# ericbrec/BSpy

Hardware: AMD Instinct MI355X
Metric: M evals/sec on 10M-point bicubic (p=3x3) surface (higher is better)
Workload: dtype f64; 1 GPU; BASELINE configs[1]: bicubic surface order 4x4, nCoef 64x64, nDep 3, fp64, clamped uniform knots, Spline.evaluate on 10000000 uniform-random (u,v); points_total=10000000, points_per_gpu=10000000, op=evaluate

## Files before the change

bspy_amd/csrc/bsk_api.hip:

```cpp
#include "bsk_kernels.hpp"
#include "bsk_tile.hpp"
#include "bsk_stream.hpp"
#include "bsk_rowrot.hpp"
#include "bsk_uniform.hpp"
#include "bsk_rec32.hpp"
#include "bsk_host.hpp"

#include <condition_variable>
#include <mutex>
#include <thread>

struct HostPipe;
static void pipe_destroy(HostPipe *p);

static int ceil_log2(int x)
{
    int s = 0;
    while ((1 << s) < x) ++s;
    return s;
}

template <typename T>
static void build_axis_table(const T *knots, int order, int nk, std::vector<T> &tab)
{
// ... 198 lines not shown
    };
#define HIPCHK_C(expr)                                                                        \
    do {                                                                                      \
        hipError_t e_ = (expr);                                                               \
        if (e_ != hipSuccess) {                                                               \
            cleanup();                                                                        \
            return fail(BSK_ERR_HIP, std::string(#expr) + ": " + hipGetErrorString(e_));      \
        }                                                                                     \
    } while (0)
    HIPCHK_C(hipSetDevice(device));
    hipDeviceProp_t prop;
    HIPCHK_C(hipGetDeviceProperties(&prop, device));
    s->num_cu = prop.multiProcessorCount > 0 ? prop.multiProcessorCount : 256;
    s->lds_max = std::min<size_t>(160 * 1024, prop.maxSharedMemoryPerMultiProcessor > 0
                                                  ? (size_t)prop.maxSharedMemoryPerMultiProcessor
                                                  : (size_t)64 * 1024);
    HIPCHK_C(hipMalloc(&s->tab, std::max<size_t>(16, s->esize * (size_t)tab_len)));
    HIPCHK_C(hipMalloc(&s->coef, std::max<size_t>(16, s->esize * (size_t)coef_len)));
    {
        const size_t tbytes = s->esize * (size_t)tab_len + s->esize * (size_t)coef_len;
        int omax = 0;
        for (int iv = 0; iv < nInd; ++iv) omax = std::max(omax, order[iv]);
        bool fixed = nInd <= 3 && omax <= 6;
        if (fixed && nDep <= 4 && tbytes + 8192 > s->lds_max)
            HIPCHK_C(hipMalloc(&s->coef_aos, std::max<size_t>(16, s->esize * (size_t)coef_len)));
        else if (fixed && nDep <= 4 && nInd == 2 && !s->same_order && omax >= 2) {
            HIPCHK_C(hipMalloc(&s->coef_aos, std::max<size_t>(16, s->esize * (size_t)coef_len)));
            s->aos_small = true;
        }
    }
    HIPCHK_C(hipMalloc((void **)&s->lut, std::max<size_t>(16, sizeof(unsigned) * (size_t)(dtype == BSK_F32 ? s->t32.lut_len : s->t64.lut_len))));
    HIPCHK_C(hipMalloc((void **)&s->bad, sizeof(unsigned long long)));
    if (const char *v = getenv("BSK_VARIANT")) s->variant = atoi(v);
    HIPCHK_C(hipMemset(s->bad, 0xff, sizeof(unsigned long long)));
#undef HIPCHK_C
    st = dtype == BSK_F32 ? upload_tables<float>(s, knots, coefs) : upload_tables<double>(s, knots, coefs);
    if (st == BSK_OK) st = dtype == BSK_F32 ? upload_uniform<float>(s, knots, coefs) : upload_uniform<double>(s, knots, coefs);
    if (st == BSK_OK) st = dtype == BSK_F32 ? upload_uniform_nd<float>(s, knots, coefs) : upload_uniform_nd<double>(s, knots, coefs);
    if (st != BSK_OK) { s->uni_img.release(); cleanup(); return st; }
    *out = s;
    return BSK_OK;
}

extern "C" bsk_status bsk_spline_update(bsk_spline s, const void *const *knots, const void *coefs)
{
    if (!s || !knots || !coefs) return fail(BSK_ERR_INVALID, "NULL argument");
    HIPCHK(hipSetDevice(s->device));
    HIPCHK(hipDeviceSynchronize());
    const bsk_status st = s->dtype == BSK_F32 ? upload_tables<float>(s, knots, coefs) : upload_tables<double>(s, knots, coefs);
    if (st != BSK_OK) return st;
    const bsk_status su = s->dtype == BSK_F32 ? upload_uniform<float>(s, knots, coefs) : upload_uniform<double>(s, knots, coefs);
    if (su != BSK_OK) return su;
    return s->dtype == BSK_F32 ? upload_uniform_nd<float>(s, knots, coefs) : upload_uniform_nd<double>(s, knots, coefs);
}

extern "C" bsk_status bsk_spline_destroy(bsk_spline s)
{
    if (!s) return BSK_OK;
    (void)hipSetDevice(s->device);
    (void)hipDeviceSynchronize();
    if (s->tab) (void)hipFree(s->tab);
    if (s->coef) (void)hipFree(s->coef);
    if (s->bad) (void)hipFree(s->bad);
    if (s->lut) (void)hipFree(s->lut);
    if (s->coef_aos) (void)hipFree(s->coef_aos);
    s->in_ws.release();
// ... 383 lines not shown
    std::vector<unsigned char> img(total_b, 0);
    for (int iv = 0; iv < nInd; ++iv)
        memcpy(img.data() + un.kn_off[iv], static_cast<const T *>(knots[iv]) + O - 1, (size_t)(un.ns[iv] + 1) * sizeof(T));
    T *ic = reinterpret_cast<T *>(img.data() + un.coef_off);
    for (size_t i = 0; i < w.size(); ++i) ic[i] = T(w[i]);
    HIPCHK(hipSetDevice(s->device));
    HIPCHK(s->uni_img.reserve(total_b));
    HIPCHK(hipMemcpy(s->uni_img.p, img.data(), total_b, hipMemcpyHostToDevice));
    s->uniN = true;
    return BSK_OK;
}

template <typename T, bool NORMAL>
static bsk_status launch_jac_rowrot(bsk_spline s, const Params<T> &prm, long long n, T *out, int normalize, int negate,
                                    hipStream_t st)
{
    const Desc<T> &d = desc_of<T>(s);
    const TileDesc<T> &tdr = tile_of<T>(s);
    const size_t lds_rr = rowrot_lds_bytes<T>(s);
    const T *tab = static_cast<const T *>(s->tab);
    const T *coef = static_cast<const T *>(s->coef);
    const int per_cu = (int)std::max<size_t>(1, std::min<size_t>(2, s->lds_max / lds_rr));
    if (s->uni) {
        const UniDesc<T> &ud = uni_of<T>(s);
        const size_t lds_u = (size_t)ud.img_bytes + TILE * sizeof(unsigned);
        const int per_cu_u = (int)std::max<size_t>(1, std::min<size_t>(2, s->lds_max / lds_u));
#define BSK_JUNI(O_, ND_)                                                                                               \
    do {                                                                                                                 \
        s->last_kernel = "jac_uni";                                        \
        HIPCHK(allow_lds(jac_uni<T, O_, NORMAL, ND_>, lds_u));                                                          \
        hipLaunchKernelGGL((jac_uni<T, O_, NORMAL, ND_>), dim3(g), dim3(TILE), lds_u, st, ud, s->uni_img.p, cp,         \
                           (unsigned)m, n0, out + n0, n, s->bad, normalize, negate);                                    \
    } while (0)
        const int ndu = (NORMAL || s->nDep > 3) ? 0 : s->nDep;
        const long long cmaxu = rr_chunk_points();
        for (long long n0 = 0; n0 < n; n0 += cmaxu) {
            const long long m = std::min<long long>(n - n0, cmaxu);
            const int g = (int)std::max<long long>(1, std::min<long long>((m + TILE - 1) / TILE, (long long)s->num_cu * per_cu_u));
            Params<T> cp = prm;
            for (int iv = 0; iv < s->nInd; ++iv) cp.p[iv] = prm.p[iv] + n0;
            if (s->order[0] == 4) {
                if constexpr (NORMAL) BSK_JUNI(4, 3);
                else switch (ndu) { case 1: BSK_JUNI(4, 1); break; case 2: BSK_JUNI(4, 2); break; case 3: BSK_JUNI(4, 3); break; default: BSK_JUNI(4, 0); }
            } else {
                if constexpr (NORMAL) BSK_JUNI(2, 3);
                else switch (ndu) { case 1: BSK_JUNI(2, 1); break; case 2: BSK_JUNI(2, 2); break; case 3: BSK_JUNI(2, 3); break; default: BSK_JUNI(2, 0); }
            }
            HIPCHK(hipGetLastError());
        }
#undef BSK_JUNI
        return BSK_OK;
    }
#define BSK_JROT(O_, ND_)                                                                                               \
    do {                                                                                                                 \
        s->last_kernel = "jac_rowrot";                                        \
        HIPCHK(allow_lds(jac_rowrot<T, O_, NORMAL, ND_>, lds_rr));                                                      \
        hipLaunchKernelGGL((jac_rowrot<T, O_, NORMAL, ND_>), dim3(g), dim3(TILE), lds_rr, st, d, tdr, tab, s->lut, coef, \
                           cp, (unsigned)m, n0, out + n0, n, s->bad, normalize, negate);                                \
    } while (0)
    const int nd = (NORMAL || s->nDep > 3) ? 0 : s->nDep;
    const long long cmax = rr_chunk_points();
    for (long long n0 = 0; n0 < n; n0 += cmax) {
        const long long m = std::min<long long>(n - n0, cmax);
        const int g = (int)std::max<long long>(1, std::min<long long>((m + TILE - 1) / TILE, (long long)s->num_cu * per_cu));
        Params<T> cp = prm;
        for (int iv = 0; iv < s->nInd; ++iv) cp.p[iv] = prm.p[iv] + n0;
        if (s->order[0] == 4) {
            if constexpr (NORMAL) BSK_JROT(4, 0);
            else switch (nd) { case 1: BSK_JROT(4, 1); break; case 2: BSK_JROT(4, 2); break; case 3: BSK_JROT(4, 3); break; default: BSK_JROT(4, 0); }
        } else {
            if constexpr (NORMAL) BSK_JROT(2, 0);
            else switch (nd) { case 1: BSK_JROT(2, 1); break; case 2: BSK_JROT(2, 2); break; case 3: BSK_JROT(2, 3); break; default: BSK_JROT(2, 0); }
        }
        HIPCHK(hipGetLastError());
    }
#undef BSK_JROT
    return BSK_OK;
}

template <typename T, int NIND, int O>
static bsk_status launch_eval_lds(bsk_spline s, size_t lds, const Params<T> &prm, long long n, T *out, long long ostride,
                                  const Wrt &w, hipStream_t st)
{
    const Desc<T> &d = desc_of<T>(s);
    const TileDesc<T> &td = tile_of<T>(s);
    const T *tab = static_cast<const T *>(s->tab);
    const T *coef = static_cast<const T *>(s->coef);
    bool deriv = false;
    for (int iv = 0; iv < s->nInd; ++iv) deriv |= w.w[iv] != 0;
    const long long ntiles = (n + TILE - 1) / TILE;
    if constexpr (NIND == 2 && (O == 2 || O == 4)) {
        if (rowrot_applies<T>(s)) {
            if (s->uni) {
                const UniDesc<T> &ud = uni_of<T>(s);
                const size_t lds_u = (size_t)ud.img_bytes + TILE * sizeof(unsigned);
                const int per_cu_u = (int)std::max<size_t>(1, std::min<size_t>(2, s->lds_max / lds_u));
#define BSK_UNI(DERIV_, ND_)                                                                                             \
    do {                                                                                                                 \
        s->last_kernel = "eval_uni";                                        \
        HIPCHK(allow_lds(eval_uni<T, O, DERIV_, ND_>, lds_u));                                                          \
        hipLaunchKernelGGL((eval_uni<T, O, DERIV_, ND_>), dim3(g), dim3(TILE), lds_u, st, ud, s->uni_img.p, cp,         \
                           (unsigned)m, n0, out + n0, ostride, w, s->bad);                                              \
    } while (0)
#define BSK_UNI_ND(DERIV_)                                                                                               \
    switch (s->nDep) {                                                                                                   \
    case 1: BSK_UNI(DERIV_, 1); break;                                                                                   \
    case 2: BSK_UNI(DERIV_, 2); break;                                                                                   \
    case 3: BSK_UNI(DERIV_, 3); break;                                                                                   \
    default: BSK_UNI(DERIV_, 0); break;                                                                                  \
    }
                const long long cmaxu = rr_chunk_points();
                for (long long n0 = 0; n0 < n; n0 += cmaxu) {
                    const long long m = std::min<long long>(n - n0, cmaxu);
                    const int g = (int)std::max<long long>(1, std::min<long long>((m + TILE - 1) / TILE, (long long)s->num_cu * per_cu_u));
                    Params<T> cp = prm;
                    for (int iv = 0; iv < s->nInd; ++iv) cp.p[iv] = prm.p[iv] + n0;
                    if (deriv) { BSK_UNI_ND(true); } else { BSK_UNI_ND(false); }
                    HIPCHK(hipGetLastError());
                }
#undef BSK_UNI_ND
#undef BSK_UNI
                return BSK_OK;
            }
            if constexpr (sizeof(T) == 4 && O == 4) {
                const size_t lds_r = r32_lds_bytes(s->ncoef[0] - 3, s->ncoef[1] - 3, td.lut_len, s->ncoef[0], s->ncoef[1]);
                if (s->variant == 0 && s->nDep >= 1 && s->nDep <= 4 && lds_r + 256 <= s->lds_max) {
                    const int per_cu_r = (int)std::max<size_t>(1, std::min<size_t>(2, s->lds_max / lds_r));
#define BSK_R32(DERIV_, ND_)                                                                                             \
    do {                                                                                                                 \
        HIPCHK(allow_lds(eval_rec32<DERIV_, ND_>, lds_r));                                                              \
        hipLaunchKernelGGL((eval_rec32<DERIV_, ND_>), dim3(g), dim3(TILE), lds_r, st, d, td, tab, s->lut, coef, cp,     \
                           (unsigned)m, n0, out + n0, ostride, w, s->bad);                                              \
    } while (0)
#define BSK_R32_ND(DERIV_)                                                                                               \
    switch (s->nDep) {                                                                                                   \
    case 1: BSK_R32(DERIV_, 1); break;                                                                                   \
    case 2: BSK_R32(DERIV_, 2); break;                                                                                   \
    case 3: BSK_R32(DERIV_, 3); break;                                                                                   \
    default: BSK_R32(DERIV_, 4); break;                                                                                  \
    }
                    s->last_kernel = "eval_rec32";
                    const long long cmaxr = rr_chunk_points();
                    for (long long n0 = 0; n0 < n; n0 += cmaxr) {
                        const long long m = std::min<long long>(n - n0, cmaxr);
                        const int g = (int)std::max<long long>(1, std::min<long long>((m + TILE - 1) / TILE, (long long)s->num_cu * per_cu_r));
                        Params<T> cp = prm;
                        for (int iv = 0; iv < s->nInd; ++iv) cp.p[iv] = prm.p[iv] + n0;
                        if (deriv) { BSK_R32_ND(true); } else { BSK_R32_ND(false); }
                        HIPCHK(hipGetLastError());
                    }
#undef BSK_R32_ND
#undef BSK_R32
                    return BSK_OK;
// ... 1341 lines not shown
```

bspy_amd/csrc/bsk_host.hpp:

```cpp
#pragma once
#include <algorithm>
#include <cmath>
#include <cstdio>
#include <cstring>
#include <limits>
#include <string>
#include <tuple>
#include <vector>

#include "bsk_common.hpp"
#include "bsk_tile.hpp"

using namespace bsk;

inline thread_local std::string g_err;

inline bsk_status fail(bsk_status st, const std::string &msg)
{
    g_err = msg;
    return st;
}

#define HIPCHK(expr)                                                                          \
    do {                                                                                      \
// ... 10 lines not shown
        if (bytes <= cap) return hipSuccess;
        if (p) (void)hipFree(p);
        p = nullptr;
        cap = 0;
        hipError_t e = hipMalloc(&p, bytes);
        if (e == hipSuccess) cap = bytes;
        return e;
    }
    void release()
    {
        if (p) (void)hipFree(p);
        p = nullptr;
        cap = 0;
    }
};

struct bsk_spline_s {
    bsk_dtype dtype;
    int device;
    int nInd, nDep;
    int order[MAXI], ncoef[MAXI];
    bool same_order;
    bool aos_small = false;
    size_t esize;
    Desc<float> d32;
    Desc<double> d64;
    TileDesc<float> t32;
    TileDesc<double> t64;
    void *tab = nullptr;
    void *coef = nullptr;
    void *coef_aos = nullptr;
    unsigned *lut = nullptr;
    int variant = 0;
    unsigned long long *bad = nullptr;
    int num_cu = 256;
    size_t lds_max = 160 * 1024;
    DevBuf in_ws, out_ws, aux_ws;
    DevBuf bin_ws;
    unsigned *ticket = nullptr;
    bool bin_reuse = false;
    DevBuf curv_ws;
    std::vector<unsigned char> tab_host;
    void *pin = nullptr;
    size_t pin_cap = 0;
    struct HostPipe *pipe = nullptr;
    bool uni = false;
    UniDesc<float> u32;
    UniDesc<double> u64;
    DevBuf uni_img;
    bool uniN = false;
    UniDescN<float> un32;
    UniDescN<double> un64;
    const char *last_kernel = "";
    static constexpr int MAX_STAGES = 12;
    bool stage_timing = false;
    hipEvent_t stage_ev[MAX_STAGES] = {};
    const char *stage_name[MAX_STAGES] = {};
    int stage_count = 0;
};

inline void stage_mark(bsk_spline s, hipStream_t st, const char *name, bool first = false)
{
    if (!s->stage_timing) return;
    if (first) s->stage_count = 0;
    if (s->stage_count >= bsk_spline_s::MAX_STAGES) return;
    hipEvent_t &e = s->stage_ev[s->stage_count];
// ... 58 lines not shown
```

bspy_amd/csrc/bsk_uniform.hpp:

```cpp
#pragma once
#include "bsk_rowrot.hpp"

namespace bsk {

__device__ __forceinline__ void stage_linear(char *smem, const void *__restrict__ gimg, unsigned bytes)
{
    const uint4 *__restrict__ g = static_cast<const uint4 *>(gimg);
    uint4 *s = reinterpret_cast<uint4 *>(smem);
    const unsigned n16 = bytes >> 4;
    constexpr int U = 8;
    const unsigned bd = blockDim.x;
    for (unsigned i0 = threadIdx.x; i0 < n16; i0 += bd * U) {
        uint4 v[U];
#pragma unroll
        for (int k = 0; k < U; ++k) v[k] = g[min(i0 + k * bd, n16 - 1u)];
#pragma unroll
        for (int k = 0; k < U; ++k) { const unsigned i = i0 + k * bd; if (i < n16) s[i] = v[k]; }
    }
}

template <typename T, bool NANFIX>
__device__ __forceinline__ void uni_spans2(const unsigned (&kn_a)[2], const UniDesc<T> &ud, const T (&u)[2], int (&m)[2],
                                           T (&z)[2])
{
    int m0[2];
    T t1[2];
#pragma unroll
    for (int iv = 0; iv < 2; ++iv) {
        const T x = (u[iv] - ud.lo[iv]) * ud.inv_h[iv] - ud.eps;
        m0[iv] = min(max((int)x, 0), ud.ns[iv] - 1);
        t1[iv] = LdsRead<T>::template at<(int)sizeof(T)>(kn_a[iv] + (unsigned)m0[iv] * (unsigned)sizeof(T));
    }
    lds_wait_n<0, 2>(t1);
#pragma unroll
    for (int iv = 0; iv < 2; ++iv) {
        const bool inc = (u[iv] >= t1[iv]) & (m0[iv] < ud.ns[iv] - 1);
        m[iv] = m0[iv] + (inc ? 1 : 0);
        z[iv] = (u[iv] - t1[iv]) * ud.inv_h[iv] + (inc ? T(0) : T(1));
        if (NANFIX && u[iv] != u[iv]) m[iv] = ud.ns[iv] - 1;
    }
}

template <typename T, int O, bool DERIV>
__device__ __forceinline__ void uni_basis(T z, int wrt, T inv_h, T (&b)[O])
{
#pragma unroll
    for (int k = 0; k < O; ++k) b[k] = T(0);
    b[O - 1] = T(1);
#pragma unroll
    for (int D = 1; D < O; ++D) {
        if (!DERIV || D < O - wrt) {
            if (D == 1) {
                b[O - 2] = T(1) - z;
                b[O - 1] = z;
            } else {
                const T rD = T(1.0 / (double)D);
#pragma unroll
                for (int j = 0; j < D; ++j) {
                    const int bi = O - D + j;
                    const T alpha = (z + T(D - 1 - j)) * rD;
                    b[bi - 1] += (T(1) - alpha) * b[bi];
                    b[bi] *= alpha;
                }
            }
        } else {
#pragma unroll
            for (int j = 0; j < D; ++j) {
                const int bi = O - D + j;
                b[bi - 1] -= inv_h * b[bi];
                b[bi] *= inv_h;
            }
        }
    }
// ... 176 lines not shown
        __builtin_amdgcn_s_setprio(3);
#pragma unroll
        for (int dep = 0; dep < nDep; ++dep) {
            T c[O][O];
            if constexpr (ND > 0) {
                uni_issue_window<T, O, ND>(ra, dep, c);
            } else {
#pragma unroll
                for (int a = 0; a < O; ++a) lds_issue_row<T, O>(ra[a], c[a]);
            }
            block_wait<0>(c);
            T q[O];
#pragma unroll
            for (int a = 0; a < O; ++a) {
                T t = T(0);
#pragma unroll
                for (int k = 0; k < O; ++k) t += c[a][k] * b[1][k];
                q[a] = mul_rn<T>(t, b0r[a]);
            }
            T r;
            if constexpr (O == 2) r = add_rn<T>(q[0], q[1]);
            else r = add_rn<T>(add_rn<T>(q[0], q[2]), add_rn<T>(q[1], q[3]));
            rr_store(o, off, r);
            o += ostride;
            if constexpr (ND == 0) {
#pragma unroll
                for (int a = 0; a < O; ++a) ra[a] += dstride;
            }
        }
        __builtin_amdgcn_s_setprio(0);
    }
}

template <typename T, int O, bool NORMAL, int ND>
__global__ __launch_bounds__(TILE) void jac_uni(const UniDesc<T> ud, const void *__restrict__ gimg, const Params<T> prm,
                                                const unsigned N, const long long n0, T *__restrict__ out,
                                                const long long ostride, unsigned long long *bad, const int normalize,
                                                const int negate)
{
    static_assert(O == 2 || O == 4, "row rotation covers orders 2 and 4");
    static_assert(!NORMAL || ND == 3, "the fused normal is a surface in 3-D");
    constexpr int CS = ND > 0 ? ND : 1;
    extern __shared__ __attribute__((aligned(16))) char smem[];
    const unsigned kn_a[2] = {(unsigned)(size_t)smem + ud.kn_off[0], (unsigned)(size_t)smem + ud.kn_off[1]};
    const unsigned coef_a = (unsigned)(size_t)smem + ud.coef_off;
    const int rs = ud.rs;
    const unsigned rstride = (unsigned)rs * (unsigned)sizeof(T);
    const unsigned dstride = (unsigned)(ud.ncoef[0] * rs) * (unsigned)sizeof(T);
    const int lane = threadIdx.x & 63;
    const unsigned stride = gridDim.x * (unsigned)TILE;
    unsigned n = ((threadIdx.x >> 6) * gridDim.x + blockIdx.x) * 64u + (unsigned)lane;
    const T lo0 = ud.lo[0], lo1 = ud.lo[1], hi0 = ud.hi[0], hi1 = ud.hi[1];
    const T *p0 = prm.p[0], *p1 = prm.p[1];
    T un[2] = {lo0, lo1};
    if (n < N) { un[0] = rr_load(p0, n * (unsigned)sizeof(T)); un[1] = rr_load(p1, n * (unsigned)sizeof(T)); }
    stage_linear(smem, gimg, ud.img_bytes);
    __syncthreads();
    unsigned *s_rc = reinterpret_cast<unsigned *>(smem + ud.img_bytes) + (threadIdx.x & ~63);
    asm volatile("" : "+v"(un[0]), "+v"(un[1]));
    const int ndep = ND > 0 ? ND : ud.nDep;

    for (; n < N; n += stride) {
        const T u[2] = {un[0], un[1]};
        const bool outside = (u[0] < lo0) | (u[0] > hi0) | (u[1] < lo1) | (u[1] > hi1);
        {
            const unsigned nn = min(n + stride, N - 1u) * (unsigned)sizeof(T);
// ... 48 lines not shown
                dv = add_rn<T>(add_rn<T>(qv[0], qv[2]), add_rn<T>(qv[1], qv[3]));
            }
            if constexpr (NORMAL) {
                if (dep == 0) { su[0] = du; sv[0] = dv; }
                else if (dep == 1) { su[1] = du; sv[1] = dv; }
                else { su[2] = du; sv[2] = dv; }
            } else {
                rr_store(o, off, du);
                rr_store(o + ostride, off, dv);
                o += 2 * ostride;
            }
            if constexpr (ND == 0) {
#pragma unroll
                for (int a = 0; a < O; ++a) ra[a] += dstride;
            }
        }
        __builtin_amdgcn_s_setprio(0);
        if constexpr (NORMAL) {
            T nx = su[1] * sv[2] - sv[1] * su[2];
            T ny = -(su[0] * sv[2] - sv[0] * su[2]);
            T nz = su[0] * sv[1] - sv[0] * su[1];
            if (negate) { nx = -nx; ny = -ny; nz = -nz; }
            if (normalize) {
                const T inv = T(1) / sqrt(nx * nx + ny * ny + nz * nz);
                nx = nx * inv; ny = ny * inv; nz = nz * inv;
            }
            rr_store(out, off, nx);
            rr_store(out + ostride, off, ny);
            rr_store(out + 2 * ostride, off, nz);
        }
    }
}

template <typename T, int NIND, bool NANFIX>
__device__ __forceinline__ void uni_spans(unsigned img_a, const UniDescN<T> &un, const T (&u)[NIND], int (&m)[NIND], T (&z)[NIND])
{
    int m0[NIND];
    T t1[NIND];
#pragma unroll
    for (int iv = 0; iv < NIND; ++iv) {
        const T x = (u[iv] - un.lo[iv]) * un.inv_h[iv] - un.eps;
        m0[iv] = min(max((int)x, 0), un.ns[iv] - 1);
        t1[iv] = LdsRead<T>::template at<(int)sizeof(T)>(img_a + un.kn_off[iv] + (unsigned)m0[iv] * (unsigned)sizeof(T));
    }
    lds_wait_n<0, NIND>(t1);
#pragma unroll
    for (int iv = 0; iv < NIND; ++iv) {
        const bool inc = (u[iv] >= t1[iv]) & (m0[iv] < un.ns[iv] - 1);
        m[iv] = m0[iv] + (inc ? 1 : 0);
        z[iv] = (u[iv] - t1[iv]) * un.inv_h[iv] + (inc ? T(0) : T(1));
        if (NANFIX && u[iv] != u[iv]) m[iv] = un.ns[iv] - 1;
    }
}

template <typename T, int NIND, int O, bool DERIV>
__global__ __launch_bounds__(STREAM_BLOCK) void eval_stream_uni(const Desc<T> d, const UniDescN<T> un, const void *__restrict__ gimg,
                                                                const Params<T> prm, const long long N, T *__restrict__ out,
                                                                const long long ostride, const Wrt wrt, unsigned long long *bad)
{
    extern __shared__ __attribute__((aligned(16))) char smem[];
    const unsigned img_a = (unsigned)(size_t)smem;
    const unsigned coef_a = img_a + un.coef_off;
    stage_linear(smem, gimg, un.img_bytes);
    __syncthreads();
    const unsigned dstride = (unsigned)d.cstride[0] * (unsigned)sizeof(T);
    const long long stride = (long long)gridDim.x * blockDim.x;
// ... 180 lines not shown
```

bspy_amd/csrc/check_lds_hazards.py:

```python
import re
import sys

KERNELS = ("eval_stream", "jac_stream", "eval_rowrot", "jac_rowrot", "curv_rowrot", "eval_uni", "jac_uni", "curv_uni",
           "eval_cellsort", "eval_slab2", "eval_rec32")
REG = re.compile(r"\bv(\d+)\b|\bv\[(\d+):(\d+)\]")
WAIT = re.compile(r"lgkmcnt\((\d+)\)")


def regs(text):
    out = set()
    for m in REG.finditer(text):
        if m.group(1) is not None:
            out.add(int(m.group(1)))
        else:
            out.update(range(int(m.group(2)), int(m.group(3)) + 1))
    return out


def lds_dest(mnem, ops):
    if mnem.startswith(("ds_read", "ds_load", "ds_bpermute", "ds_permute", "ds_swizzle", "ds_consume", "ds_append")) \
            or "_rtn" in mnem:
        return regs(ops.split(",")[0])
    return set()


def used_regs(mnem, ops):
    if not mnem.startswith("v_pk_") or not mnem.endswith("f32"):
        return regs(ops)
    fields = [f.strip() for f in re.split(r",(?![^\[]*\])", ops.split(" op_sel")[0].split(" neg_")[0])]
    sel = {"op_sel": None, "op_sel_hi": None}
    for key in sel:
        m = re.search(key + r":\[([01,]+)\]", ops)
        if m:
            sel[key] = [int(x) for x in m.group(1).split(",")]
    out = regs(fields[0])
    for i, f in enumerate(fields[1:]):
        m = re.fullmatch(r"v\[(\d+):(\d+)\]", f)
        if not m:
            out |= regs(f)
            continue
        lo = int(m.group(1))
        a = sel["op_sel"][i] if sel["op_sel"] and i < len(sel["op_sel"]) else 0
        b = sel["op_sel_hi"][i] if sel["op_sel_hi"] and i < len(sel["op_sel_hi"]) else 1
        out |= {lo + a, lo + b}
    return out


def split_blocks(lines):
    blocks = [{"labels": [], "insts": []}]
    for ln, raw in lines:
        text = raw.split(";")[0].strip()
        if not text or text.startswith("//") or (text.startswith(".") and not text.endswith(":")):
            continue
        if text.endswith(":"):
            if blocks[-1]["insts"]:
                blocks.append({"labels": [], "insts": []})
            blocks[-1]["labels"].append(text[:-1])
            continue
        parts = text.split(None, 1)
        mnem, ops = parts[0], (parts[1] if len(parts) > 1 else "")
        blocks[-1]["insts"].append((ln, mnem, ops, text))
        if mnem.startswith(("s_cbranch", "s_branch", "s_endpgm", "s_setpc")):
            blocks.append({"labels": [], "insts": []})
    index = {lab: i for i, b in enumerate(blocks) for lab in b["labels"]}
    for i, b in enumerate(blocks):
        succ = []
        last = b["insts"][-1] if b["insts"] else None
        if last and last[1].startswith("s_cbranch"):
            succ = [index.get(last[2].strip()), i + 1]
        elif last and last[1] == "s_branch":
            succ = [index.get(last[2].strip())]
        elif last and last[1].startswith(("s_endpgm", "s_setpc")):
            succ = []
        else:
            succ = [i + 1]
        b["succ"] = [x for x in succ if x is not None and x < len(blocks)]
    return blocks


def run_block(block, fifo, errors=None):
    for ln, mnem, ops, text in block["insts"]:
        if mnem == "s_waitcnt":
            m = WAIT.search(ops)
            if m:
                keep = int(m.group(1))
                fifo = () if keep == 0 else (fifo[-keep:] if len(fifo) > keep else fifo)
            elif "cnt" not in ops:
                try:
                    if int(ops, 0) == 0:
                        fifo = ()
                except ValueError:
                    pass
            continue
        if errors is not None:
            used = used_regs(mnem, ops)
            for dest, dln, dtext in fifo:
                hit = set(dest) & used
                if hit:
                    errors.append((ln, f"{text}   touches v{sorted(hit)[0]} of the LDS read still in flight",
                                   f"line {dln}: {dtext}"))
                    break
        if mnem.startswith("ds_"):
            fifo = fifo + ((tuple(sorted(lds_dest(mnem, ops))), ln, text),)
        elif mnem.startswith(("s_load", "s_buffer_load", "s_memtime", "s_memrealtime")):
            fifo = fifo + (((), ln, text),)
        while len(fifo) > 16 and not fifo[0][0]:
            fifo = fifo[1:]
    return fifo


def covers(long, short):
    if len(long) < len(short):
        return False
    if not any(f[0] for f in long) and not any(f[0] for f in short):
        return True
    return not short or long[len(long) - len(short):] == short


MAX_STATES = 32


def merge(states, out):
    if states is None:
        return (out,)
    if any(covers(st, out) for st in states):
        return states
    return tuple(st for st in states if not covers(out, st)) + (out,)


def check_kernel(name, lines):
    errors = []
    blocks = split_blocks(lines)
    state = [None] * len(blocks)
    state[0] = ((),)
    work = [0]
    rounds = 0
    while work and not errors:
        rounds += 1
        if rounds > 100000:
            errors.append((0, "data-flow did not converge", ""))
            break
        i = work.pop()
        for st in state[i]:
            out = run_block(blocks[i], st)
            if len(out) > 64:
                errors.append((blocks[i]["insts"][0][0], "LDS operations pile up along a loop (never awaited)", ""))
                break
            for j in blocks[i]["succ"]:
                m = merge(state[j], out)
                if len(m) > MAX_STATES:
                    ln = blocks[j]["insts"][0][0] if blocks[j]["insts"] else 0
                    errors.append((ln, "too many unrelated sets of outstanding LDS reads reach " + "/".join(blocks[j]["labels"]), ""))
                    break
                if m != state[j]:
                    state[j] = m
                    if j not in work:
                        work.append(j)
            if errors:
                break
    if not errors:
        for b, sts in zip(blocks, state):
            for st in sts or ():
                run_block(b, st, errors)
        errors = sorted(set(errors))
    return errors


def main():
    args = [a for a in sys.argv[1:] if a != "--allow-none"]
    allow_none = "--allow-none" in sys.argv[1:]
    path = args[0]
    wanted = tuple(args[1:]) or KERNELS
    kernels = {}
    cur = None
    with open(path) as f:
        for ln, raw in enumerate(f, 1):
            if cur is None:
                m = re.match(r"^(_Z\w+):", raw)
                if m and any(re.search(k, m.group(1)) for k in wanted):
                    cur = m.group(1)
                    kernels[cur] = []
                continue
            kernels[cur].append((ln, raw))
            if "s_endpgm" in raw.split(";")[0]:
                cur = None
    if not kernels:
        print("check_lds_hazards: no asm-LDS kernel found in", path)
        return 0 if allow_none else 1
    bad = 0
    for name, lines in kernels.items():
        errs = check_kernel(name, lines)
        for ln, what, where in errs[:5]:
            print(f"LDS HAZARD in {name}\n  line {ln}: {what}\n  {where}", flush=True)
        bad += len(errs)
    if bad:
        print(f"check_lds_hazards: {bad} hazard(s) in {len(kernels)} kernels")
        return 1
    print(f"no LDS read hazards in {len(kernels)} asm-LDS kernels")
    return 0


if __name__ == "__main__":
    sys.exit(main())
```

Baseline: 113,700 M evals/s.

## Software-pipeline uniform-knot eval and jacobian kernels with prefetched parameters and spans

Adds pipelined variants of the uniform-knot evaluate and jacobian kernels. Each thread prefetches (u,v) parameters several iterations ahead using inline global loads with counted vmcnt waits. It also overlaps the next point's span lookup and LDS rank atomic with the current point's coefficient reads and FMAs. The aim is to hide global load latency and LDS round-trips that the plain kernel exposes on every point. In exchange it relies on hand-counted wait counts that must match the store count per iteration, raises register pressure, and extends the hazard checker to cover global loads. The old path stays reachable through BSK_VARIANT=10.

```diff
diff --git a/bspy_amd/csrc/bsk_api.hip b/bspy_amd/csrc/bsk_api.hip
--- a/bspy_amd/csrc/bsk_api.hip
+++ b/bspy_amd/csrc/bsk_api.hip
@@ -254,6 +254,7 @@
     HIPCHK_C(hipMalloc((void **)&s->lut, std::max<size_t>(16, sizeof(unsigned) * (size_t)(dtype == BSK_F32 ? s->t32.lut_len : s->t64.lut_len))));
     HIPCHK_C(hipMalloc((void **)&s->bad, sizeof(unsigned long long)));
     if (const char *v = getenv("BSK_VARIANT")) s->variant = atoi(v);
+    if (s->variant == 10) { s->variant = 0; s->uni_plain = true; }
     HIPCHK_C(hipMemset(s->bad, 0xff, sizeof(unsigned long long)));
 #undef HIPCHK_C
     st = dtype == BSK_F32 ? upload_tables<float>(s, knots, coefs) : upload_tables<double>(s, knots, coefs);
@@ -703,6 +704,18 @@
         hipLaunchKernelGGL((jac_uni<T, O_, NORMAL, ND_>), dim3(g), dim3(TILE), lds_u, st, ud, s->uni_img.p, cp,         \
                            (unsigned)m, n0, out + n0, n, s->bad, normalize, negate);                                    \
     } while (0)
+#define BSK_JUNI_PIPE(O_, ND_)                                                                                          \
+    do {                                                                                                                 \
+         \
+        if constexpr (NORMAL && sizeof(T) == 4) { BSK_JUNI(O_, ND_); break; }                                            \
+        else {                                                                                                           \
+            if (s->uni_plain) { BSK_JUNI(O_, ND_); break; }                                                          \
+            s->last_kernel = "jac_uni";                                                                                  \
+            HIPCHK(allow_lds(jac_uni_pipe<T, O_, NORMAL, ND_>, lds_u));                                                 \
+            hipLaunchKernelGGL((jac_uni_pipe<T, O_, NORMAL, ND_>), dim3(g), dim3(TILE), lds_u, st, ud, s->uni_img.p, cp, \
+                               (unsigned)m, n0, out + n0, n, s->bad, normalize, negate);                                \
+        }                                                                                                                \
+    } while (0)
         const int ndu = (NORMAL || s->nDep > 3) ? 0 : s->nDep;
         const long long cmaxu = rr_chunk_points();
         for (long long n0 = 0; n0 < n; n0 += cmaxu) {
@@ -711,14 +724,15 @@
             Params<T> cp = prm;
             for (int iv = 0; iv < s->nInd; ++iv) cp.p[iv] = prm.p[iv] + n0;
             if (s->order[0] == 4) {
-                if constexpr (NORMAL) BSK_JUNI(4, 3);
-                else switch (ndu) { case 1: BSK_JUNI(4, 1); break; case 2: BSK_JUNI(4, 2); break; case 3: BSK_JUNI(4, 3); break; default: BSK_JUNI(4, 0); }
+                if constexpr (NORMAL) BSK_JUNI_PIPE(4, 3);
+                else switch (ndu) { case 1: BSK_JUNI_PIPE(4, 1); break; case 2: BSK_JUNI_PIPE(4, 2); break; case 3: BSK_JUNI_PIPE(4, 3); break; default: BSK_JUNI(4, 0); }
             } else {
-                if constexpr (NORMAL) BSK_JUNI(2, 3);
-                else switch (ndu) { case 1: BSK_JUNI(2, 1); break; case 2: BSK_JUNI(2, 2); break; case 3: BSK_JUNI(2, 3); break; default: BSK_JUNI(2, 0); }
+                if constexpr (NORMAL) BSK_JUNI_PIPE(2, 3);
+                else switch (ndu) { case 1: BSK_JUNI_PIPE(2, 1); break; case 2: BSK_JUNI_PIPE(2, 2); break; case 3: BSK_JUNI_PIPE(2, 3); break; default: BSK_JUNI(2, 0); }
             }
             HIPCHK(hipGetLastError());
         }
+#undef BSK_JUNI_PIPE
 #undef BSK_JUNI
         return BSK_OK;
     }
@@ -773,11 +787,19 @@
         hipLaunchKernelGGL((eval_uni<T, O, DERIV_, ND_>), dim3(g), dim3(TILE), lds_u, st, ud, s->uni_img.p, cp,         \
                            (unsigned)m, n0, out + n0, ostride, w, s->bad);                                              \
     } while (0)
+#define BSK_UNI_PIPE(DERIV_, ND_)                                                                                        \
+    do {                                                                                                                 \
+        if (s->uni_plain) { BSK_UNI(DERIV_, ND_); break; }                                                           \
+        s->last_kernel = "eval_uni";                 \
+        HIPCHK(allow_lds(eval_uni_pipe<T, O, DERIV_, ND_>, lds_u));                                                     \
+        hipLaunchKernelGGL((eval_uni_pipe<T, O, DERIV_, ND_>), dim3(g), dim3(TILE), lds_u, st, ud, s->uni_img.p, cp,    \
+                           (unsigned)m, n0, out + n0, ostride, w, s->bad);                                              \
+    } while (0)
 #define BSK_UNI_ND(DERIV_)                                                                                               \
     switch (s->nDep) {                                                                                                   \
-    case 1: BSK_UNI(DERIV_, 1); break;                                                                                   \
-    case 2: BSK_UNI(DERIV_, 2); break;                                                                                   \
-    case 3: BSK_UNI(DERIV_, 3); break;                                                                                   \
+    case 1: BSK_UNI_PIPE(DERIV_, 1); break;                                                                              \
+    case 2: BSK_UNI_PIPE(DERIV_, 2); break;                                                                              \
+    case 3: BSK_UNI_PIPE(DERIV_, 3); break;                                                                              \
     default: BSK_UNI(DERIV_, 0); break;                                                                                  \
     }
                 const long long cmaxu = rr_chunk_points();
@@ -790,6 +812,7 @@
                     HIPCHK(hipGetLastError());
                 }
 #undef BSK_UNI_ND
+#undef BSK_UNI_PIPE
 #undef BSK_UNI
                 return BSK_OK;
             }
diff --git a/bspy_amd/csrc/bsk_host.hpp b/bspy_amd/csrc/bsk_host.hpp
--- a/bspy_amd/csrc/bsk_host.hpp
+++ b/bspy_amd/csrc/bsk_host.hpp
@@ -66,6 +66,7 @@
     void *coef_aos = nullptr;
     unsigned *lut = nullptr;
     int variant = 0;
+    bool uni_plain = false;
     unsigned long long *bad = nullptr;
     int num_cu = 256;
     size_t lds_max = 160 * 1024;
diff --git a/bspy_amd/csrc/bsk_uniform.hpp b/bspy_amd/csrc/bsk_uniform.hpp
--- a/bspy_amd/csrc/bsk_uniform.hpp
+++ b/bspy_amd/csrc/bsk_uniform.hpp
@@ -19,19 +19,21 @@
     }
 }
 
-template <typename T, bool NANFIX>
-__device__ __forceinline__ void uni_spans2(const unsigned (&kn_a)[2], const UniDesc<T> &ud, const T (&u)[2], int (&m)[2],
-                                           T (&z)[2])
-{
-    int m0[2];
-    T t1[2];
+template <typename T>
+__device__ __forceinline__ void uni_spans2_issue(const unsigned (&kn_a)[2], const UniDesc<T> &ud, const T (&u)[2], int (&m0)[2],
+                                                 T (&t1)[2])
+{
 #pragma unroll
     for (int iv = 0; iv < 2; ++iv) {
         const T x = (u[iv] - ud.lo[iv]) * ud.inv_h[iv] - ud.eps;
         m0[iv] = min(max((int)x, 0), ud.ns[iv] - 1);
         t1[iv] = LdsRead<T>::template at<(int)sizeof(T)>(kn_a[iv] + (unsigned)m0[iv] * (unsigned)sizeof(T));
     }
-    lds_wait_n<0, 2>(t1);
+}
+template <typename T, bool NANFIX>
+__device__ __forceinline__ void uni_spans2_decide(const UniDesc<T> &ud, const T (&u)[2], const int (&m0)[2], const T (&t1)[2],
+                                                  int (&m)[2], T (&z)[2])
+{
 #pragma unroll
     for (int iv = 0; iv < 2; ++iv) {
         const bool inc = (u[iv] >= t1[iv]) & (m0[iv] < ud.ns[iv] - 1);
@@ -39,6 +41,16 @@
         z[iv] = (u[iv] - t1[iv]) * ud.inv_h[iv] + (inc ? T(0) : T(1));
         if (NANFIX && u[iv] != u[iv]) m[iv] = ud.ns[iv] - 1;
     }
+}
+template <typename T, bool NANFIX>
+__device__ __forceinline__ void uni_spans2(const unsigned (&kn_a)[2], const UniDesc<T> &ud, const T (&u)[2], int (&m)[2],
+                                           T (&z)[2])
+{
+    int m0[2];
+    T t1[2];
+    uni_spans2_issue<T>(kn_a, ud, u, m0, t1);
+    lds_wait_n<0, 2>(t1);
+    uni_spans2_decide<T, NANFIX>(ud, u, m0, t1, m, z);
 }
 
 template <typename T, int O, bool DERIV>
@@ -281,6 +293,195 @@
     }
 }
 
+template <typename T>
+struct GlobalLoad;
+template <>
+struct GlobalLoad<double> {
+    static __device__ __forceinline__ double at(const double *base, unsigned byte_off)
+    {
+        double v;
+        asm volatile("global_load_dwordx2 %0, %1, %2" : "=v"(v) : "v"(byte_off), "s"(base) : "memory");
+        return v;
+    }
+};
+template <>
+struct GlobalLoad<float> {
+    static __device__ __forceinline__ float at(const float *base, unsigned byte_off)
+    {
+        float v;
+        asm volatile("global_load_dword %0, %1, %2" : "=v"(v) : "v"(byte_off), "s"(base) : "memory");
+        return v;
+    }
+};
+template <int CNT, typename T>
+__device__ __forceinline__ void vm_wait_pair(T (&v)[2])
+{
+    static_assert(CNT >= 0 && CNT <= 63, "vmcnt is 6 bits");
+    asm volatile("s_waitcnt vmcnt(%2)" : "+v"(v[0]), "+v"(v[1]) : "n"(CNT) : "memory");
+}
+
+template <typename T>
+struct UniFront {
+    T z[2];
+    int base;
+    int rank;
+    int outside;
+};
+
+template <typename T>
+struct UniLoop {
+    unsigned kn_a[2], coef_a, rc_a;
+    int rs, lane;
+    unsigned rstride, stride, last;
+    T lo0, lo1, hi0, hi1;
+    const T *p0, *p1;
+};
+
+template <typename T>
+__device__ __forceinline__ void uni_load_params(const UniLoop<T> &L, unsigned n, T (&un)[2])
+{
+    const unsigned nn = min(n, L.last) * (unsigned)sizeof(T);
+    un[0] = GlobalLoad<T>::at(L.p0, nn);
+    un[1] = GlobalLoad<T>::at(L.p1, nn);
+}
+
+template <typename T, int O, bool NANFIX, int CS>
+__device__ __forceinline__ void uni_front_finish(const UniDesc<T> &ud, const UniLoop<T> &L, const T (&u)[2], const int (&m0)[2],
+                                                 const T (&t1)[2], UniFront<T> &f)
+{
+    int m[2];
+    uni_spans2_decide<T, NANFIX>(ud, u, m0, t1, m, f.z);
+    f.outside = ((u[0] < L.lo0) | (u[0] > L.hi0) | (u[1] < L.lo1) | (u[1] > L.hi1)) ? 1 : 0;
+    f.base = (int)__umul24((unsigned)m[0], (unsigned)L.rs) + m[1] * CS;
+    asm volatile("" : "+v"(f.z[0]), "+v"(f.z[1]), "+v"(f.base), "+v"(f.outside));
+    const unsigned a = L.rc_a + 4u * (unsigned)((L.lane & 32) + (f.base & (32 / O - 1)));
+    asm volatile("ds_add_rtn_u32 %0, %1, %2" : "=v"(f.rank) : "v"(a), "v"(1u) : "memory");
+}
+__device__ __forceinline__ void uni_rank_wait(int &rank)
+{
+    asm volatile("s_waitcnt lgkmcnt(0)" : "+v"(rank) : : "memory");
+}
+
+template <typename T>
+__device__ __forceinline__ void uni_loop_setup(UniLoop<T> &L, char *smem, const UniDesc<T> &ud, const Params<T> &prm, unsigned N)
+{
+    L.kn_a[0] = (unsigned)(size_t)smem + ud.kn_off[0];
+    L.kn_a[1] = (unsigned)(size_t)smem + ud.kn_off[1];
+    L.coef_a = (unsigned)(size_t)smem + ud.coef_off;
+    L.rc_a = (unsigned)(size_t)smem + ud.img_bytes + 4u * (threadIdx.x & ~63u);
+    L.rs = ud.rs;
+    L.lane = threadIdx.x & 63;
+    L.rstride = (unsigned)ud.rs * (unsigned)sizeof(T);
+    L.stride = gridDim.x * (unsigned)TILE;
+    L.last = N - 1u;
+    L.lo0 = ud.lo[0]; L.lo1 = ud.lo[1]; L.hi0 = ud.hi[0]; L.hi1 = ud.hi[1];
+    L.p0 = prm.p[0]; L.p1 = prm.p[1];
+}
+
+template <typename T, int O, bool NANFIX, int CS>
+__device__ __forceinline__ void uni_pipe_prologue(const UniDesc<T> &ud, const UniLoop<T> &L, char *smem, const void *__restrict__ gimg,
+                                                  unsigned n, T (&u0)[2], T (&ua)[2], T (&ub)[2], UniFront<T> &f)
+{
+    uni_load_params<T>(L, n, u0);
+    uni_load_params<T>(L, n + L.stride, ua);
+    uni_load_params<T>(L, n + 2u * L.stride, ub);
+    stage_linear(smem, gimg, ud.img_bytes);
+    __syncthreads();
+    vm_wait_pair<0>(u0);
+    vm_wait_pair<0>(ua);
+    vm_wait_pair<0>(ub);
+    int m0[2];
+    T t1[2];
+    uni_spans2_issue<T>(L.kn_a, ud, u0, m0, t1);
+    lds_wait_n<0, 2>(t1);
+    uni_front_finish<T, O, NANFIX, CS>(ud, L, u0, m0, t1, f);
+    uni_rank_wait(f.rank);
+}
+
+template <typename T, int O, bool DERIV, int ND, bool LAST = false>
+__device__ __forceinline__ void eval_uni_step(const UniDesc<T> &ud, const UniLoop<T> &L, unsigned n, const long long n0, T *out,
+                                              const long long ostride, const Wrt &wrt, unsigned long long *bad, UniFront<T> &f,
+                                              T (&un)[2])
+{
+    if (f.outside) {
+        record_bad(bad, n0 + (long long)n);
+        asm volatile("s_waitcnt vmcnt(0)" : : : "memory");
+    }
+    T b[2][O];
+    if constexpr (!DERIV) {
+        uni_basis_closed<T, O>(f.z[0], b[0]);
+        uni_basis_closed<T, O>(f.z[1], b[1]);
+    } else {
+        uni_basis<T, O, true>(f.z[0], wrt.w[0], ud.inv_h[0], b[0]);
+        uni_basis<T, O, true>(f.z[1], wrt.w[1], ud.inv_h[1], b[1]);
+    }
+    unsigned ra[O];
+    const int rho = uni_rows<T, O>(L.coef_a, f.base, f.rank, L.rstride, ra);
+    T b0r[O];
+    rotate_basis_values<T, O>(b[0], rho, b0r);
+
+    if constexpr (!LAST) vm_wait_pair<2 * ND + 1>(un);
+    int m0[2];
+    T t1[2];
+    const unsigned off = n * (unsigned)sizeof(T);
+    T *o = out;
+    __builtin_amdgcn_s_setprio(3);
+#pragma unroll
+    for (int dep = 0; dep < ND; ++dep) {
+        T c[O][O];
+        uni_issue_window<T, O, ND>(ra, dep, c);
+        if (dep == 0 && !LAST) {
+            uni_spans2_issue<T>(L.kn_a, ud, un, m0, t1);
+            block_wait<2>(c);
+        } else {
+            block_wait<0>(c);
+        }
+        T q[O];
+#pragma unroll
+        for (int a = 0; a < O; ++a) {
+            T t = T(0);
+#pragma unroll
+            for (int k = 0; k < O; ++k) t += c[a][k] * b[1][k];
+            q[a] = mul_rn<T>(t, b0r[a]);
+        }
+        T r;
+        if constexpr (O == 2) r = add_rn<T>(q[0], q[1]);
+        else r = add_rn<T>(add_rn<T>(q[0], q[2]), add_rn<T>(q[1], q[3]));
+        rr_store(o, off, r);
+        o += ostride;
+        if (dep == 0 && !LAST) {
+            lds_wait_n<0, 2>(t1);
+            uni_front_finish<T, O, DERIV, ND>(ud, L, un, m0, t1, f);
+            uni_load_params<T>(L, n + 3u * L.stride, un);
+        }
+    }
+    __builtin_amdgcn_s_setprio(0);
+    if constexpr (!LAST) uni_rank_wait(f.rank);
+}
+
+template <typename T, int O, bool DERIV, int ND>
+__global__ __launch_bounds__(TILE) void eval_uni_pipe(const UniDesc<T> ud, const void *__restrict__ gimg, const Params<T> prm,
+                                                      const unsigned N, const long long n0, T *__restrict__ out,
+                                                      const long long ostride, const Wrt wrt, unsigned long long *bad)
+{
+    static_assert(O == 2 || O == 4, "row rotation covers orders 2 and 4");
+    static_assert(ND >= 1 && ND <= 3, "counted vmcnt: the store count per iteration is a constant");
+    extern __shared__ __attribute__((aligned(16))) char smem[];
+    UniLoop<T> L;
+    uni_loop_setup<T>(L, smem, ud, prm, N);
+    unsigned n = ((threadIdx.x >> 6) * gridDim.x + blockIdx.x) * 64u + (unsigned)L.lane;
+    T u0[2], ua[2], ub[2];
+    UniFront<T> f;
+    uni_pipe_prologue<T, O, DERIV, ND>(ud, L, smem, gimg, n, u0, ua, ub, f);
+    for (; n + L.stride < N; n += 2u * L.stride) {
+        eval_uni_step<T, O, DERIV, ND>(ud, L, n, n0, out, ostride, wrt, bad, f, ua);
+        eval_uni_step<T, O, DERIV, ND>(ud, L, n + L.stride, n0, out, ostride, wrt, bad, f, ub);
+    }
+    vm_wait_pair<ND - 1>(ua);
+    vm_wait_pair<ND - 1>(ub);
+    if (n < N) eval_uni_step<T, O, DERIV, ND, true>(ud, L, n, n0, out, ostride, wrt, bad, f, ua);
+}
+
 template <typename T, int O, bool NORMAL, int ND>
 __global__ __launch_bounds__(TILE) void jac_uni(const UniDesc<T> ud, const void *__restrict__ gimg, const Params<T> prm,
                                                 const unsigned N, const long long n0, T *__restrict__ out,
@@ -395,6 +596,119 @@
     }
 }
 
+template <bool NORMAL, int ND>
+struct JacUniCounts {
+    static constexpr int tail = NORMAL ? 3 : 2 * ND - 2;
+    static constexpr int slot = NORMAL ? 8 : 4 * ND;
+};
+template <typename T, int O, bool NORMAL, int ND, bool LAST = false>
+__device__ __forceinline__ void jac_uni_step(const UniDesc<T> &ud, const UniLoop<T> &L, unsigned n, const long long n0, T *out,
+                                             const long long ostride, unsigned long long *bad, const int normalize,
+                                             const int negate, UniFront<T> &f, T (&un)[2])
+{
+    if (f.outside) {
+        record_bad(bad, n0 + (long long)n);
+        asm volatile("s_waitcnt vmcnt(0)" : : : "memory");
+    }
+    T b[2][O], db[2][O];
+    uni_basis_d1<T, O>(f.z[0], ud.inv_h[0], b[0], db[0]);
+    uni_basis_d1<T, O>(f.z[1], ud.inv_h[1], b[1], db[1]);
+    unsigned ra[O];
+    const int rho = uni_rows<T, O>(L.coef_a, f.base, f.rank, L.rstride, ra);
+    T b0r[O], db0r[O];
+    rotate_basis_values<T, O>(b[0], rho, b0r);
+    rotate_basis_values<T, O>(db[0], rho, db0r);
+
+    if constexpr (!LAST) vm_wait_pair<JacUniCounts<NORMAL, ND>::slot>(un);
+    int m0[2];
+    T t1[2];
+    const unsigned off = n * (unsigned)sizeof(T);
+    T *o = out;
+    T su[3], sv[3];
+    __builtin_amdgcn_s_setprio(3);
+#pragma unroll
+    for (int dep = 0; dep < ND; ++dep) {
+        T c[O][O];
+        uni_issue_window<T, O, ND>(ra, dep, c);
+        if (dep == 0 && !LAST) {
+            uni_spans2_issue<T>(L.kn_a, ud, un, m0, t1);
+            block_wait<2>(c);
+        } else {
+            block_wait<0>(c);
+        }
+        T qu[O], qv[O];
+#pragma unroll
+        for (int a = 0; a < O; ++a) {
+            T t = T(0), tdv = T(0);
+#pragma unroll
+            for (int k = 0; k < O; ++k) { t += c[a][k] * b[1][k]; tdv += c[a][k] * db[1][k]; }
+            qu[a] = mul_rn<T>(t, db0r[a]);
+            qv[a] = mul_rn<T>(tdv, b0r[a]);
+        }
+        T du, dv;
+        if constexpr (O == 2) {
+            du = add_rn<T>(qu[0], qu[1]);
+            dv = add_rn<T>(qv[0], qv[1]);
+        } else {
+            du = add_rn<T>(add_rn<T>(qu[0], qu[2]), add_rn<T>(qu[1], qu[3]));
+            dv = add_rn<T>(add_rn<T>(qv[0], qv[2]), add_rn<T>(qv[1], qv[3]));
+        }
+        if constexpr (NORMAL) {
+            if (dep == 0) { su[0] = du; sv[0] = dv; }
+            else if (dep == 1) { su[1] = du; sv[1] = dv; }
+            else { su[2] = du; sv[2] = dv; }
+        } else {
+            rr_store(o, off, du);
+            rr_store(o + ostride, off, dv);
+            o += 2 * ostride;
+        }
+        if (dep == 0 && !LAST) {
+            lds_wait_n<0, 2>(t1);
+            uni_front_finish<T, O, true, ND>(ud, L, un, m0, t1, f);
+            uni_load_params<T>(L, n + 3u * L.stride, un);
+        }
+    }
+    __builtin_amdgcn_s_setprio(0);
+    if constexpr (!LAST) uni_rank_wait(f.rank);
+    if constexpr (NORMAL) {
+        T nx = su[1] * sv[2] - sv[1] * su[2];
+        T ny = -(su[0] * sv[2] - sv[0] * su[2]);
+        T nz = su[0] * sv[1] - sv[0] * su[1];
+        if (negate) { nx = -nx; ny = -ny; nz = -nz; }
+        if (normalize) {
+            const T inv = T(1) / sqrt(nx * nx + ny * ny + nz * nz);
+            nx = nx * inv; ny = ny * inv; nz = nz * inv;
+        }
+        rr_store(out, off, nx);
+        rr_store(out + ostride, off, ny);
+        rr_store(out + 2 * ostride, off, nz);
+    }
+}
+
+template <typename T, int O, bool NORMAL, int ND>
+__global__ __launch_bounds__(TILE) void jac_uni_pipe(const UniDesc<T> ud, const void *__restrict__ gimg, const Params<T> prm,
+                                                     const unsigned N, const long long n0, T *__restrict__ out,
+                                                     const long long ostride, unsigned long long *bad, const int normalize,
+                                                     const int negate)
+{
+    static_assert(O == 2 || O == 4, "row rotation covers orders 2 and 4");
+    static_assert(ND >= 1 && ND <= 3 && (!NORMAL || ND == 3), "counted vmcnt: the store count per iteration is a constant");
+    extern __shared__ __attribute__((aligned(16))) char smem[];
+    UniLoop<T> L;
+    uni_loop_setup<T>(L, smem, ud, prm, N);
+    unsigned n = ((threadIdx.x >> 6) * gridDim.x + blockIdx.x) * 64u + (unsigned)L.lane;
+    T u0[2], ua[2], ub[2];
+    UniFront<T> f;
+    uni_pipe_prologue<T, O, true, ND>(ud, L, smem, gimg, n, u0, ua, ub, f);
+    for (; n + L.stride < N; n += 2u * L.stride) {
+        jac_uni_step<T, O, NORMAL, ND>(ud, L, n, n0, out, ostride, bad, normalize, negate, f, ua);
+        jac_uni_step<T, O, NORMAL, ND>(ud, L, n + L.stride, n0, out, ostride, bad, normalize, negate, f, ub);
+    }
+    vm_wait_pair<JacUniCounts<NORMAL, ND>::tail>(ua);
+    vm_wait_pair<JacUniCounts<NORMAL, ND>::tail>(ub);
+    if (n < N) jac_uni_step<T, O, NORMAL, ND, true>(ud, L, n, n0, out, ostride, bad, normalize, negate, f, ua);
+}
+
 template <typename T, int NIND, bool NANFIX>
 __device__ __forceinline__ void uni_spans(unsigned img_a, const UniDescN<T> &un, const T (&u)[NIND], int (&m)[NIND], T (&z)[NIND])
 {
diff --git a/bspy_amd/csrc/check_lds_hazards.py b/bspy_amd/csrc/check_lds_hazards.py
--- a/bspy_amd/csrc/check_lds_hazards.py
+++ b/bspy_amd/csrc/check_lds_hazards.py
@@ -4,7 +4,18 @@
 KERNELS = ("eval_stream", "jac_stream", "eval_rowrot", "jac_rowrot", "curv_rowrot", "eval_uni", "jac_uni", "curv_uni",
            "eval_cellsort", "eval_slab2", "eval_rec32")
 REG = re.compile(r"\bv(\d+)\b|\bv\[(\d+):(\d+)\]")
-WAIT = re.compile(r"lgkmcnt\((\d+)\)")
+
+
+class Counter:
+
+    def __init__(self, name, width, what):
+        self.name, self.cap, self.what = name, width, what
+        self.wait = re.compile(name + r"\((\d+)\)")
+
+
+LGKM = Counter("lgkmcnt", 16, "LDS read")
+VM = Counter("vmcnt", 64, "global load")
+VMEM = ("global_", "buffer_", "flat_", "scratch_")
 
 
 def regs(text):
@@ -20,6 +31,14 @@
 def lds_dest(mnem, ops):
     if mnem.startswith(("ds_read", "ds_load", "ds_bpermute", "ds_permute", "ds_swizzle", "ds_consume", "ds_append")) \
             or "_rtn" in mnem:
+        return regs(ops.split(",")[0])
+    return set()
+
+
+def vm_dest(mnem, ops):
+    if "_load" in mnem and not mnem.endswith("_lds") and " lds" not in ops:
+        return regs(ops.split(",")[0])
+    if "_atomic" in mnem and re.search(r"\b(glc|sc0)\b", ops):
         return regs(ops.split(",")[0])
     return set()
 
@@ -78,10 +97,10 @@
     return blocks
 
 
-def run_block(block, fifo, errors=None):
+def run_block(block, fifo, errors=None, ctr=LGKM):
     for ln, mnem, ops, text in block["insts"]:
         if mnem == "s_waitcnt":
-            m = WAIT.search(ops)
+            m = ctr.wait.search(ops)
             if m:
                 keep = int(m.group(1))
                 fifo = () if keep == 0 else (fifo[-keep:] if len(fifo) > keep else fifo)
@@ -97,14 +116,17 @@
             for dest, dln, dtext in fifo:
                 hit = set(dest) & used
                 if hit:
-                    errors.append((ln, f"{text}   touches v{sorted(hit)[0]} of the LDS read still in flight",
+                    errors.append((ln, f"{text}   touches v{sorted(hit)[0]} of the {ctr.what} still in flight",
                                    f"line {dln}: {dtext}"))
                     break
-        if mnem.startswith("ds_"):
+        if ctr is VM:
+            if mnem.startswith(VMEM):
+                fifo = fifo + ((tuple(sorted(vm_dest(mnem, ops))), ln, text),)
+        elif mnem.startswith("ds_"):
             fifo = fifo + ((tuple(sorted(lds_dest(mnem, ops))), ln, text),)
         elif mnem.startswith(("s_load", "s_buffer_load", "s_memtime", "s_memrealtime")):
             fifo = fifo + (((), ln, text),)
-        while len(fifo) > 16 and not fifo[0][0]:
+        while len(fifo) > ctr.cap and not fifo[0][0]:
             fifo = fifo[1:]
     return fifo
 
@@ -128,7 +150,7 @@
     return tuple(st for st in states if not covers(out, st)) + (out,)
 
 
-def check_kernel(name, lines):
+def check_kernel(name, lines, ctr=LGKM):
     errors = []
     blocks = split_blocks(lines)
     state = [None] * len(blocks)
@@ -142,15 +164,15 @@
             break
         i = work.pop()
         for st in state[i]:
-            out = run_block(blocks[i], st)
-            if len(out) > 64:
-                errors.append((blocks[i]["insts"][0][0], "LDS operations pile up along a loop (never awaited)", ""))
+            out = run_block(blocks[i], st, None, ctr)
+            if len(out) > 4 * ctr.cap:
+                errors.append((blocks[i]["insts"][0][0], f"{ctr.what}s pile up along a loop (never awaited)", ""))
                 break
             for j in blocks[i]["succ"]:
                 m = merge(state[j], out)
                 if len(m) > MAX_STATES:
                     ln = blocks[j]["insts"][0][0] if blocks[j]["insts"] else 0
-                    errors.append((ln, "too many unrelated sets of outstanding LDS reads reach " + "/".join(blocks[j]["labels"]), ""))
+                    errors.append((ln, f"too many unrelated sets of outstanding {ctr.what}s reach " + "/".join(blocks[j]["labels"]), ""))
                     break
                 if m != state[j]:
                     state[j] = m
@@ -161,9 +183,21 @@
     if not errors:
         for b, sts in zip(blocks, state):
             for st in sts or ():
-                run_block(b, st, errors)
+                run_block(b, st, errors, ctr)
         errors = sorted(set(errors))
     return errors
+
+
+def has_asm_vmem(lines):
+    inside = False
+    for _, raw in lines:
+        if "#ASMSTART" in raw:
+            inside = True
+        elif "#ASMEND" in raw:
+            inside = False
+        elif inside and raw.split(";")[0].strip().startswith(VMEM):
+            return True
+    return False
 
 
 def main():
@@ -181,22 +215,26 @@
                     cur = m.group(1)
                     kernels[cur] = []
                 continue
+            if raw.startswith(".Lfunc_end"):
+                cur = None
+                continue
             kernels[cur].append((ln, raw))
-            if "s_endpgm" in raw.split(";")[0]:
-                cur = None
     if not kernels:
         print("check_lds_hazards: no asm-LDS kernel found in", path)
         return 0 if allow_none else 1
-    bad = 0
+    bad = n_vm = 0
     for name, lines in kernels.items():
         errs = check_kernel(name, lines)
+        if has_asm_vmem(lines):
+            n_vm += 1
+            errs += check_kernel(name, lines, VM)
         for ln, what, where in errs[:5]:
             print(f"LDS HAZARD in {name}\n  line {ln}: {what}\n  {where}", flush=True)
         bad += len(errs)
     if bad:
         print(f"check_lds_hazards: {bad} hazard(s) in {len(kernels)} kernels")
         return 1
-    print(f"no LDS read hazards in {len(kernels)} asm-LDS kernels")
+    print(f"no LDS read hazards in {len(kernels)} asm-LDS kernels" + (f", no global load hazards in {n_vm} of them" if n_vm else ""))
     return 0
 
 
```

Result: slower. 111,100 M evals/s (-2.3%).
